# gongweibao/FleetX

Hardware: AMD Instinct MI355X
Metric: tokens/sec (whole node) GPT-3 6.7B hybrid-parallel at 1/2/4/8 MI355X (higher is better)
Workload: dtype bf16; 1 GPU; model=gpt3-6.7B, global_batch=8, seq_len=1024, parallelism=dp1, micro_batch=8, hip_graph=True, grad_reduce_dtype=float32, recompute=False

## Files before the change

csrc/kernels/norm_eltwise.hip:

```cpp
#include "fx_api.h"
#include "fx_common.h"

namespace {

struct DropCfg {
  uint32_t klo, khi, thr;
  float scale;
  int enabled;
  const uint64_t* salt;
};

__device__ __forceinline__ DropCfg resolve_drop(DropCfg d) {
  if (d.enabled && d.salt != nullptr) {
    const uint64_t k = salt_key(((uint64_t)d.khi << 32) | d.klo, *d.salt);
    d.klo = (uint32_t)k;
    d.khi = (uint32_t)(k >> 32);
  }
  return d;
}

__device__ __forceinline__ float drop_apply(float v, uint64_t idx, const DropCfg& d) {
  if (!d.enabled) return v;
  uint32_t h = elem_rand_pair(idx, d.klo, d.khi);
  uint32_t r = (idx & 1) ? (h >> 16) : (h & 0xffffu);
// ... 287 lines not shown
    const uint16_t* __restrict__ gamma, const uint16_t* __restrict__ ds_in,
    uint16_t* __restrict__ ds_out, uint16_t* __restrict__ dx_out, int rows, int h,
    int rows_per_group, float* __restrict__ part, DropCfg drop_) {
  constexpr int NG = 4 / WPR;
  __shared__ float red[4 * 512 * VPT];
  __shared__ float xs[2][4][2];
  const DropCfg drop = resolve_drop(drop_);
  const int lane = threadIdx.x & 63, w = threadIdx.x >> 6;
  const int grp = w / WPR, half = w % WPR;
  const int hw = h / WPR, cbase = half * hw;
  const int r0 = min(rows, (blockIdx.x * NG + grp) * rows_per_group);
  const int r1 = min(rows, r0 + rows_per_group);
  uint4 gp[VPT];
  float ag[VPT][8], ab[VPT][8], ax[DB ? VPT : 1][8];
#pragma unroll
  for (int i = 0; i < VPT; ++i) {
    const int c = (i * 64 + lane) * 8;
    gp[i] = (!MASK || c < hw) ? *reinterpret_cast<const uint4*>(gamma + cbase + c)
                              : make_uint4(0, 0, 0, 0);
#pragma unroll
    for (int j = 0; j < 8; ++j) {
      ag[i][j] = ab[i][j] = 0.f;
      if (DB) ax[i][j] = 0.f;
    }
  }
  for (int k = 0; k < rows_per_group; ++k) {
    const int r = r0 + k;
    const bool live = r < r1;
    if (WPR == 1 && !live) break;
    const size_t base = (size_t)(live ? r : 0) * h + cbase;
    uint4 ca[VPT], cd[VPT], cr[VPT];
    float mean = 0.f, rstd = 0.f, s1 = 0.f, s2 = 0.f;
    if (live) {
#pragma unroll
      for (int i = 0; i < VPT; ++i) {
        const int c = (i * 64 + lane) * 8;
        if (MASK && c >= hw) continue;
        ca[i] = *reinterpret_cast<const uint4*>(s + base + c);
        cd[i] = *reinterpret_cast<const uint4*>(dy + base + c);
      }
      if (ds_in) {
#pragma unroll
        for (int i = 0; i < VPT; ++i) {
          const int c = (i * 64 + lane) * 8;
          if (MASK && c >= hw) continue;
          cr[i] = *reinterpret_cast<const uint4*>(ds_in + base + c);
        }
      }
      mean = mean_in[r];
      rstd = rstd_in[r];
#pragma unroll
      for (int i = 0; i < VPT; ++i) {
        const int c = (i * 64 + lane) * 8;
        if (MASK && c >= hw) continue;
        float a[8], d[8], g[8];
        unpack8<T>(ca[i], a);
        unpack8<T>(cd[i], d);
        unpack8<T>(gp[i], g);
#pragma unroll
        for (int j = 0; j < 8; ++j) {
          const float xh = (a[j] - mean) * rstd, gd = d[j] * g[j];
          s1 += gd;
          s2 += gd * xh;
          ag[i][j] += d[j] * xh;
          ab[i][j] += d[j];
        }
      }
    }
    s1 = wave_sum(s1);
    s2 = wave_sum(s2);
    if constexpr (WPR > 1) {
      if (lane == 0) {
        xs[k & 1][w][0] = s1;
        xs[k & 1][w][1] = s2;
      }
      __syncthreads();
      s1 = xs[k & 1][WPR * grp][0];
      s2 = xs[k & 1][WPR * grp][1];
#pragma unroll
      for (int q = 1; q < WPR; ++q) {
        s1 += xs[k & 1][WPR * grp + q][0];
        s2 += xs[k & 1][WPR * grp + q][1];
      }
    }
    if (!live) continue;
    const float m1 = s1 / h, m2 = s2 / h;
#pragma unroll
    for (int i = 0; i < VPT; ++i) {
      const int c = (i * 64 + lane) * 8;
      if (MASK && c >= hw) continue;
      float a[8], d[8], g[8], o[8];
      unpack8<T>(ca[i], a);
      unpack8<T>(cd[i], d);
      unpack8<T>(gp[i], g);
#pragma unroll
      for (int j = 0; j < 8; ++j) o[j] = rstd * (d[j] * g[j] - m1 - (a[j] - mean) * rstd * m2);
      if (ds_in) {
        float rr[8];
        unpack8<T>(cr[i], rr);
#pragma unroll
        for (int j = 0; j < 8; ++j) o[j] += rr[j];
      }
      store8<T>(ds_out + base + c, o);
      if (drop.enabled) {
        drop_apply8(o, base + c, drop);
        store8<T>(dx_out + base + c, o);
      } else if (dx_out != ds_out) {
        store8<T>(dx_out + base + c, o);
      }
      if (DB) {
#pragma unroll
        for (int j = 0; j < 8; ++j) ax[i][j] += round_to<T>(o[j]);
      }
    }
  }
#pragma unroll
  for (int arr = 0; arr < (DB ? 3 : 2); ++arr) {
    __syncthreads();
#pragma unroll
    for (int i = 0; i < VPT; ++i) {
      const int c = (i * 64 + lane) * 8;
      if (MASK && c >= hw) continue;
#pragma unroll
      for (int j = 0; j < 8; ++j)
        red[grp * h + cbase + c + j] = arr == 0 ? ag[i][j] : arr == 1 ? ab[i][j] : ax[DB ? i : 0][j];
    }
    __syncthreads();
    float* out = part + ((size_t)arr * gridDim.x + blockIdx.x) * h;
    for (int c = threadIdx.x; c < h; c += 256) {
      float v = red[c];
#pragma unroll
      for (int q = 1; q < NG; ++q) v += red[q * h + c];
      out[c] = v;
    }
  }
}

struct LnColsOut {
  float* f32[3];
  uint16_t* t16[3];
  int acc[3];
};
template <typename T>
__global__ __launch_bounds__(256) void ln_cols_finalize_kernel(const float* __restrict__ part,
                                                               int G, int h, LnColsOut f) {
  __shared__ float tr[8][132];
  const int arr = blockIdx.y;
  const float* p = part + (size_t)arr * G * h;
  const int q = threadIdx.x & 31, sr = threadIdx.x >> 5;
  const int c0 = blockIdx.x * 128 + q * 4;
  floatx4 acc = {0.f, 0.f, 0.f, 0.f};
  if (c0 < h) {
    for (int k0 = sr; k0 < G; k0 += 128) {
      floatx4 v[16];
#pragma unroll
      for (int u = 0; u < 16; ++u) {
        const int k = k0 + 8 * u;
        v[u] = k < G ? *reinterpret_cast<const floatx4*>(p + (size_t)k * h + c0)
                     : floatx4{0.f, 0.f, 0.f, 0.f};
      }
#pragma unroll
      for (int u = 0; u < 16; ++u) acc += v[u];
    }
  }
#pragma unroll
  for (int j = 0; j < 4; ++j) tr[sr][q * 4 + j] = acc[j];
// ... 438 lines not shown
    }
#undef LNM_CASE
  } else {
    FX_DISPATCH_T(dtype, add_ln_fwd_generic<T><<<grid, block, 0, st>>>(
                             X, B, R, G, Be, S, Y, mean, rstd, rows, h, eps, d));
  }
#undef LN_CASE
}

extern "C" void fx_ln_bwd_row(int dtype, const void* dy, const void* s, const float* mean,
                              const float* rstd, const void* gamma, const void* ds_in,
                              void* ds_out, void* dx_out, int rows, int h, float p, uint64_t key,
                              const void* salt, hipStream_t st) {
  DropCfg d = make_drop(p, key, salt);
  dim3 grid((rows + 3) / 4), block(256);
  auto DY = (const uint16_t*)dy;
  auto S = (const uint16_t*)s;
  auto G = (const uint16_t*)gamma;
  auto DI = (const uint16_t*)ds_in;
  auto DS = (uint16_t*)ds_out;
  auto DX = (uint16_t*)dx_out;
#define LNB_CASE(V)                                                                       \
  case V:                                                                                 \
    FX_DISPATCH_T(dtype, ln_bwd_row_kernel<T, V><<<grid, block, 0, st>>>(                 \
                             DY, S, mean, rstd, G, DI, DS, DX, rows, h, d));              \
    break;
  if (h % 512 == 0 && h / 512 <= 8) {
    switch (h / 512) {
      LNB_CASE(1) LNB_CASE(2) LNB_CASE(3) LNB_CASE(4) LNB_CASE(5) LNB_CASE(6) LNB_CASE(7)
      LNB_CASE(8)
      default:
        FX_DISPATCH_T(dtype, ln_bwd_row_generic<T><<<grid, block, 0, st>>>(
                                 DY, S, mean, rstd, G, DI, DS, DX, rows, h, d));
    }
  } else if (h % 8 == 0 && h < 8 * 512) {
#define LNBM_CASE(V)                                                                      \
  case V:                                                                                 \
    FX_DISPATCH_T(dtype, ln_bwd_row_kernel<T, V, true><<<grid, block, 0, st>>>(           \
                             DY, S, mean, rstd, G, DI, DS, DX, rows, h, d));              \
    break;
    switch ((h + 511) / 512) {
      LNBM_CASE(1) LNBM_CASE(2) LNBM_CASE(3) LNBM_CASE(4) LNBM_CASE(5) LNBM_CASE(6)
      LNBM_CASE(7) LNBM_CASE(8)
    }
#undef LNBM_CASE
  } else {
    FX_DISPATCH_T(dtype, ln_bwd_row_generic<T><<<grid, block, 0, st>>>(
                             DY, S, mean, rstd, G, DI, DS, DX, rows, h, d));
  }
#undef LNB_CASE
}

static int ln_cols_wpr(int h) { return h <= 1536 ? 1 : h <= 3072 ? 2 : 4; }
static int ln_cols_rows_per_group(int rows, int h) {
  const int ng = 4 / ln_cols_wpr(h);
  int rpg = (rows + 512 * ng - 1) / (512 * ng);
  return rpg < 2 ? 2 : rpg;
}
extern "C" int fx_ln_bwd_cols_blocks(int rows, int h, int max_h) {
  if (rows <= 0 || h > (max_h < 4096 ? max_h : 4096) || h % (8 * ln_cols_wpr(h))) return 0;
  const int ng = 4 / ln_cols_wpr(h), rpg = ln_cols_rows_per_group(rows, h);
  return (rows + ng * rpg - 1) / (ng * rpg);
}

extern "C" int fx_ln_bwd_cols(int dtype, const void* dy, const void* s, const float* mean,
                              const float* rstd, const void* gamma, const void* ds_in,
                              void* ds_out, void* dx_out, int rows, int h, float p, uint64_t key,
                              float* part, int with_dbias, float* fg, void* tg, int accg,
                              float* fb, void* tb, int accb, float* fx, void* tx, int accx,
                              const void* salt, hipStream_t st) {
  const int G = fx_ln_bwd_cols_blocks(rows, h, 4096);
  if (G == 0) return -1;
  const int wpr = ln_cols_wpr(h), hw = h / wpr;
  const int rpg = ln_cols_rows_per_group(rows, h);
  DropCfg d = make_drop(p, key, salt);
  auto DY = (const uint16_t*)dy;
  auto S = (const uint16_t*)s;
  auto GM = (const uint16_t*)gamma;
  auto DI = (const uint16_t*)ds_in;
  auto DS = (uint16_t*)ds_out;
  auto DX = (uint16_t*)dx_out;
  const int vpt = (hw + 511) / 512;
  const bool mask = hw % 512 != 0;
#define LNC_GO(V, W, M, DB)                                                                   \
  FX_DISPATCH_T(dtype, ln_bwd_cols_kernel<T, V, W, M, DB><<<G, 256, 0, st>>>(                 \
                           DY, S, mean, rstd, GM, DI, DS, DX, rows, h, rpg, part, d))
#define LNC_M(V, W)                                                                           \
  if (mask) {                                                                                 \
    if (with_dbias) { LNC_GO(V, W, true, true); } else { LNC_GO(V, W, true, false); }         \
  } else {                                                                                    \
    if (with_dbias) { LNC_GO(V, W, false, true); } else { LNC_GO(V, W, false, false); }       \
  }
#define LNC_V(V)                                                                              \
  case V:                                                                                     \
    if (wpr == 1) { LNC_M(V, 1) } else if (wpr == 2) { LNC_M(V, 2) } else { LNC_M(V, 4) }     \
    break;
  switch (vpt) {
    LNC_V(1) LNC_V(2) LNC_V(3)
    default: return -1;
  }
#undef LNC_V
#undef LNC_M
#undef LNC_GO
  LnColsOut f;
  f.f32[0] = fg; f.f32[1] = fb; f.f32[2] = fx;
  f.t16[0] = (uint16_t*)tg; f.t16[1] = (uint16_t*)tb; f.t16[2] = (uint16_t*)tx;
  f.acc[0] = accg; f.acc[1] = accb; f.acc[2] = accx;
  dim3 grid((h + 127) / 128, with_dbias ? 3 : 2);
  FX_DISPATCH_T(dtype, ln_cols_finalize_kernel<T><<<grid, 256, 0, st>>>(part, G, h, f));
  return 0;
}

extern "C" void fx_coltile_partial(int dtype, int mode, const void* a, const void* b,
                                   const float* mean, const float* rstd, float* p0, float* p1,
                                   int rows, int cols, int splits, hipStream_t st, int* cnt,
                                   float* f0, void* t0, int acc0, float* f1, void* t1, int acc1) {
  const ColFin fin = make_fin(cnt, f0, t0, acc0, f1, t1, acc1);
  int rps = (rows + splits - 1) / splits;
  dim3 grid((cols + 127) / 128, splits), block(256);
  auto A = (const uint16_t*)a;
  auto B = (const uint16_t*)b;
  if (mode == 0) {
    FX_DISPATCH_T(dtype, coltile_partial_kernel<T, 0><<<grid, block, 0, st>>>(
                             A, B, mean, rstd, p0, p1, rows, cols, rps, fin));
  } else {
    FX_DISPATCH_T(dtype, coltile_partial_kernel<T, 1><<<grid, block, 0, st>>>(
                             A, B, mean, rstd, p0, p1, rows, cols, rps, fin));
  }
}

extern "C" void fx_coltile_finalize(int dtype, const float* part, int splits, int cols,
                                    float* out_f32, void* out_t, int accumulate, hipStream_t st) {
  dim3 grid((cols + 255) / 256), block(256);
  FX_DISPATCH_T(dtype, coltile_finalize_kernel<T><<<grid, block, 0, st>>>(
                           part, splits, cols, out_f32, (uint16_t*)out_t, accumulate));
}

extern "C" void fx_bias_gelu_fwd(int dtype, int erf, const void* x, const void* bias, void* y,
                                 long n, int cols, hipStream_t st) {
  long n8 = n / 8;
  if (erf) {
    FX_DISPATCH_T(dtype, bias_gelu_fwd_kernel<T, true><<<grid_for(n8), 256, 0, st>>>(
                             (const uint16_t*)x, (const uint16_t*)bias, (uint16_t*)y, n8, cols));
  } else {
    FX_DISPATCH_T(dtype, bias_gelu_fwd_kernel<T, false><<<grid_for(n8), 256, 0, st>>>(
                             (const uint16_t*)x, (const uint16_t*)bias, (uint16_t*)y, n8, cols));
  }
}

extern "C" void fx_bias_gelu_bwd(int dtype, int erf, const void* dy, const void* x,
                                 const void* bias, void* dx, float* part, int rows, int cols,
                                 int splits, hipStream_t st, int* cnt, float* out_f32,
                                 void* out_t, int acc) {
  const ColFin fin = make_fin(cnt, out_f32, out_t, acc, nullptr, nullptr, 0);
  int rps = (rows + splits - 1) / splits;
  dim3 grid((cols + 127) / 128, splits), block(256);
  if (erf) {
    FX_DISPATCH_T(dtype, bias_gelu_bwd_kernel<T, true><<<grid, block, 0, st>>>(
                             (const uint16_t*)dy, (const uint16_t*)x, (const uint16_t*)bias,
                             (uint16_t*)dx, part, rows, cols, rps, fin));
  } else {
    FX_DISPATCH_T(dtype, bias_gelu_bwd_kernel<T, false><<<grid, block, 0, st>>>(
                             (const uint16_t*)dy, (const uint16_t*)x, (const uint16_t*)bias,
                             (uint16_t*)dx, part, rows, cols, rps, fin));
  }
}

extern "C" void fx_bias_dropout_add_fwd(int dtype, const void* x, const void* bias,
                                        const void* residual, void* out, long n, int cols, float p,
                                        uint64_t key, const void* salt, hipStream_t st) {
  DropCfg d = make_drop(p, key, salt);
  long n8 = n / 8;
  FX_DISPATCH_T(dtype, bias_dropout_add_fwd_kernel<T><<<grid_for(n8), 256, 0, st>>>(
                           (const uint16_t*)x, (const uint16_t*)bias, (const uint16_t*)residual,
                           (uint16_t*)out, n8, cols, d));
}

extern "C" void fx_dropout_bwd_colsum(int dtype, const void* dout, void* dx, float* part,
                                      int rows, int cols, int splits, float p, uint64_t key,
                                      const void* salt, hipStream_t st, int* cnt,
                                      float* out_f32, void* out_t, int acc) {
  const ColFin fin = make_fin(cnt, out_f32, out_t, acc, nullptr, nullptr, 0);
  DropCfg d = make_drop(p, key, salt);
  int rps = (rows + splits - 1) / splits;
  dim3 grid((cols + 127) / 128, splits), block(256);
  FX_DISPATCH_T(dtype, dropout_bwd_colsum_kernel<T><<<grid, block, 0, st>>>(
// ... 11 lines not shown
```

fleetx_amd/models/language_model/gpt/model.py:

```python
import math

import torch
import torch.nn as nn

from .... import ops
from ....parallel import layers as L
from ....parallel import mappings as M
from ....parallel import topology as topo
from ....parallel.linear import fused_mlp
from ....parallel.recompute import recompute
from ....parallel.rng import get_rng_state_tracker


class GPTConfig:
    def __init__(self, vocab_size=50304, hidden_size=1024, num_layers=24, num_attention_heads=16,
                 ffn_hidden_size=None, hidden_dropout_prob=0.1, attention_probs_dropout_prob=0.1,
                 max_position_embeddings=1024, type_vocab_size=16, initializer_range=0.02,
                 use_recompute=False, recompute_granularity=None, sequence_parallel=False,
                 layer_norm_eps=1e-5, fused_linear=False, no_recompute_layers=None,
                 fused_lm_head_ce=False, dtype=torch.float32, **unused):
        self.vocab_size = vocab_size
        self.hidden_size = hidden_size
        self.num_layers = num_layers
        self.num_attention_heads = num_attention_heads
        self.ffn_hidden_size = ffn_hidden_size or 4 * hidden_size
        self.hidden_dropout_prob = hidden_dropout_prob
        self.attention_probs_dropout_prob = attention_probs_dropout_prob
        self.max_position_embeddings = max_position_embeddings
        self.type_vocab_size = type_vocab_size
        self.initializer_range = initializer_range
        self.use_recompute = use_recompute
        self.recompute_granularity = recompute_granularity or ("full" if use_recompute else None)
        self.sequence_parallel = sequence_parallel and topo.mp_world_size() > 1
        self.layer_norm_eps = layer_norm_eps
        self.no_recompute_layers = set(no_recompute_layers or [])
        self.dtype = dtype
        self.head_dim = hidden_size // num_attention_heads
        self.fused_lm_head_ce = bool(fused_lm_head_ce)

    @classmethod
    def from_model_config(cls, cfg, dtype=torch.float32):
        keys = ["vocab_size", "hidden_size", "num_layers", "num_attention_heads", "ffn_hidden_size",
                "hidden_dropout_prob", "attention_probs_dropout_prob", "max_position_embeddings",
                "type_vocab_size", "initializer_range", "use_recompute", "recompute_granularity",
                "sequence_parallel", "no_recompute_layers", "layer_norm_eps", "fused_lm_head_ce"]
        kw = {k: cfg[k] for k in keys if k in cfg and cfg[k] is not None}
        return cls(dtype=dtype, **kw)


def _key(stream):
    return get_rng_state_tracker().next_key(stream)


class GPTEmbeddings(nn.Module):
    def __init__(self, cfg):
        super().__init__()
        self.cfg = cfg
        self.word_embeddings = L.VocabParallelEmbedding(cfg.vocab_size, cfg.hidden_size,
                                                        std=cfg.initializer_range,
                                                        name="embeddings.word", dtype=cfg.dtype)
        self.position_embeddings = nn.Parameter(L.init_full_then_slice(
            (cfg.max_position_embeddings, cfg.hidden_size), cfg.initializer_range,
            "embeddings.position", dtype=cfg.dtype))
        self.position_embeddings.sequence_parallel = cfg.sequence_parallel

    def forward(self, input_ids, position_ids=None):
        b, s = input_ids.shape
        if position_ids is None:
            position_ids = torch.arange(s, device=input_ids.device).unsqueeze(0).expand(b, s)
        sp = self.cfg.sequence_parallel
        if sp:
            input_ids = input_ids.t()
            position_ids = position_ids.t()
        if topo.mp_world_size() == 1:
            x = ops.embedding(input_ids, self.word_embeddings.weight, position_ids,
                              self.position_embeddings, 0)
        else:
            x = self.word_embeddings(input_ids)
            if sp:
                x = M.reduce_scatter_seq(x)
                pos = ops.embedding(M._split(position_ids, topo.mp_group(), 0),
                                    self.position_embeddings)
            else:
                x = M.reduce_from_mp(x)
                pos = ops.embedding(position_ids, self.position_embeddings)
            x = x + pos
        p = self.cfg.hidden_dropout_prob if self.training else 0.0
        if p > 0:
            x = ops.dropout(x, p, _key("local_seed" if sp else "global_seed"))
        return x


class GPTAttention(nn.Module):
    def __init__(self, cfg, idx):
        super().__init__()
        self.cfg = cfg
        t = topo.mp_world_size()
        assert cfg.num_attention_heads % t == 0
        self.heads = cfg.num_attention_heads // t
        self.head_dim = cfg.head_dim
        std = cfg.initializer_range
        self.qkv_proj = L.ColumnParallelLinear(cfg.hidden_size, 3 * cfg.hidden_size, bias=True,
                                               sequence_parallel=cfg.sequence_parallel, std=std,
                                               name="layers.%d.attn.qkv" % idx, dtype=cfg.dtype)
        self.out_proj = L.RowParallelLinear(cfg.hidden_size, cfg.hidden_size, bias=True,
                                            skip_bias_add=True,
                                            sequence_parallel=cfg.sequence_parallel, std=std,
                                            name="layers.%d.attn.out" % idx, dtype=cfg.dtype)

    def core_attn(self, qkv, key):
        cfg = self.cfg
        p = cfg.attention_probs_dropout_prob if self.training else 0.0
        if cfg.sequence_parallel:
            s, b = qkv.shape[0], qkv.shape[1]
            qkv5 = qkv.view(s, b, self.heads, 3, self.head_dim).transpose(0, 1)
        else:
            b, s = qkv.shape[0], qkv.shape[1]
            qkv5 = qkv.view(b, s, self.heads, 3, self.head_dim)
        o = ops.flash_attention_qkvpacked(qkv5, causal=True, dropout_p=p, key=key)
        if cfg.sequence_parallel:
            return o.transpose(0, 1).reshape(s, b, self.heads * self.head_dim)
        return o.reshape(b, s, self.heads * self.head_dim)

    def forward(self, x):
        qkv = self.qkv_proj(x)
        key = _key("local_seed") if (self.training and self.cfg.attention_probs_dropout_prob > 0) else 0
        if self.cfg.recompute_granularity == "core_attn" and self.training:
            o = recompute(self.core_attn, qkv, key)
        else:
            o = self.core_attn(qkv, key)
        return self.out_proj(o)


class GPTMLP(nn.Module):
    def __init__(self, cfg, idx):
        super().__init__()
        std = cfg.initializer_range
        self.fc1 = L.ColumnParallelLinear(cfg.hidden_size, cfg.ffn_hidden_size, bias=True,
                                          skip_bias_add=True,
                                          sequence_parallel=cfg.sequence_parallel, std=std,
                                          name="layers.%d.mlp.fc1" % idx, dtype=cfg.dtype)
        self.fc2 = L.RowParallelLinear(cfg.ffn_hidden_size, cfg.hidden_size, bias=True,
                                       skip_bias_add=True, sequence_parallel=cfg.sequence_parallel,
                                       std=std, name="layers.%d.mlp.fc2" % idx, dtype=cfg.dtype)
        self.fc1.sp_chunk_major = self.fc2.sp_chunk_major = bool(cfg.sequence_parallel)

    def forward(self, x):
        if topo.mp_world_size() == 1 and type(self.fc1) is L.ColumnParallelLinear \
                and type(self.fc2) is L.RowParallelLinear:
            return fused_mlp(x, self.fc1.weight, self.fc1.bias, self.fc2.weight), self.fc2.bias
        y, b = self.fc1(x)
        y = ops.bias_gelu(y, b, approximate=True)
        return self.fc2(y)


class GPTDecoderLayer(nn.Module):

    def __init__(self, cfg, idx):
        super().__init__()
        self.cfg = cfg
        self.idx = idx
        self.ln1 = ops.FusedLayerNorm(cfg.hidden_size, cfg.layer_norm_eps, dtype=cfg.dtype)
        self.attn = GPTAttention(cfg, idx)
        self.ln2 = ops.FusedLayerNorm(cfg.hidden_size, cfg.layer_norm_eps, dtype=cfg.dtype)
        self.mlp = GPTMLP(cfg, idx)
        if cfg.sequence_parallel:
            L.mark_sequence_parallel(self.ln1)
            L.mark_sequence_parallel(self.ln2)

    def _attn_block(self, x):
        return self.attn(self.ln1(x))

    def _attn_block_out(self, x):
        return self._attn_block(x)[0]

    def _forward(self, x):
        cfg = self.cfg
        p = cfg.hidden_dropout_prob if self.training else 0.0
        stream = "local_seed" if cfg.sequence_parallel else "global_seed"
        if cfg.recompute_granularity == "full_attn" and self.training:
            a, ab = recompute(self._attn_block_out, x), self.attn.out_proj.bias
        else:
            x, h1 = ops.layer_norm_keep_input(x, self.ln1.weight, self.ln1.bias, self.ln1.eps)
            a, ab = self.attn(h1)
        k1 = _key(stream) if p > 0 else 0
        x2, h2 = ops.add_layer_norm(a, ab, x, self.ln2.weight, self.ln2.bias, self.ln2.eps, p, k1)
        m, mb = self.mlp(h2)
        k2 = _key(stream) if p > 0 else 0
        return ops.bias_dropout_add(m, mb, x2, p, k2)

    def forward(self, x):
        if (self.cfg.recompute_granularity == "full" and self.training
                and self.idx not in self.cfg.no_recompute_layers):
            return recompute(self._forward, x)
        return self._forward(x)


class GPTModel(nn.Module):

    def __init__(self, cfg, layer_range=None, has_embedding=True, has_final_ln=True):
        super().__init__()
        self.cfg = cfg
        start, end = layer_range if layer_range is not None else (0, cfg.num_layers)
        self.embeddings = GPTEmbeddings(cfg) if has_embedding else None
        self.layers = nn.ModuleList([GPTDecoderLayer(cfg, i) for i in range(start, end)])
        self.final_ln = ops.FusedLayerNorm(cfg.hidden_size, cfg.layer_norm_eps,
                                           dtype=cfg.dtype) if has_final_ln else None
        if has_final_ln and cfg.sequence_parallel:
            L.mark_sequence_parallel(self.final_ln)

    def forward(self, input_ids=None, position_ids=None, hidden=None):
        x = self.embeddings(input_ids, position_ids) if self.embeddings is not None else hidden
        for layer in self.layers:
            x = layer(x)
        if self.final_ln is not None:
            x = self.final_ln(x)
        return x


class GPTForPretraining(nn.Module):

    def __init__(self, cfg):
        super().__init__()
        self.cfg = cfg
        self.gpt = GPTModel(cfg)
        emb = self.gpt.embeddings
        if emb is not None:
            emb.word_embeddings.weight._fx_fused_wgrad_ok = True
            emb.word_embeddings.weight._fx_grad_parts = 2
            emb.position_embeddings._fx_fused_wgrad_ok = True

    def forward(self, input_ids, position_ids=None):
        h = self.gpt(input_ids, position_ids)
        w = self.gpt.embeddings.word_embeddings.weight
        if self.cfg.fused_lm_head_ce and self.training:
            return L.parallel_lm_head_input(h, w, sequence_parallel=self.cfg.sequence_parallel)
        logits = L.parallel_lm_logits(h, w, parallel_output=True,
                                      sequence_parallel=self.cfg.sequence_parallel)
        return logits


class GPTPretrainingCriterion(nn.Module):

    def __init__(self, cfg=None):
        super().__init__()
        self.seq_first = bool(cfg is not None and cfg.sequence_parallel)

    def forward(self, logits, labels, loss_mask):
        if self.seq_first:
            labels, loss_mask = labels.t(), loss_mask.t()
        g = topo.get_hcg().get_model_parallel_group()
        if isinstance(logits, L.HeadInput):
            from ....parallel.linear import linear
            from ....ops import lm_head_ce
            hi = logits
            vocab_start = topo.mp_rank() * hi.weight.shape[0]
            if lm_head_ce.supported(hi.h2, hi.weight):
                return lm_head_ce.lm_head_cross_entropy(
                    hi.h2, hi.weight, labels.reshape(-1), loss_mask.reshape(-1),
                    group=g if g.nranks > 1 else None, vocab_start=vocab_start)
            logits = linear(hi.h2, hi.weight)
        vocab_start = topo.mp_rank() * logits.shape[-1]
        ce = ops.softmax_cross_entropy(logits, labels, group=g if g.nranks > 1 else None,
                                       vocab_start=vocab_start)
        mask = loss_mask.reshape(-1).float()
        return (ce.reshape(-1) * mask).sum() / mask.sum()


def num_params(cfg):
    l, h, V, s = cfg.num_layers, cfg.hidden_size, cfg.vocab_size, cfg.max_position_embeddings
    return 12 * l * h * h * (1 + 13.0 / (12 * h) + (V + s) / (12.0 * l * h))


def flops_per_token(cfg, seq_len):
    l, h, V = cfg.num_layers, cfg.hidden_size, cfg.vocab_size
    return 72.0 * l * h * h * (1 + seq_len / (6.0 * h) + V / (12.0 * h * l))
```

fleetx_amd/ops/norm.py:

```python
import os

import torch

from . import _lib
from ..parallel import grad_sink as sink, rng as _rng


_TICKETS = {}


def colsum_tickets(device, cols):
    st = torch.cuda.current_stream(device).cuda_stream
    need = 32 * ((cols + 127) // 128)
    t = _TICKETS.get(st)
    if t is None or t.numel() < need:
        t = torch.zeros(max(4096, need), dtype=torch.int32, device=device)
        _TICKETS[st] = t
    return t.data_ptr()


_TARGET_KW = (("f0", "t0", "acc0"), ("f1", "t1", "acc1"))


def _coltile(mode, x, aux, rows, cols, targets):
    k = _lib.kernels()
    splits = k.coltile_splits(rows, cols)
    p0 = torch.empty(splits, cols, device=x.device, dtype=torch.float32)
    p1 = torch.empty_like(p0) if mode == 0 else None
    fin = {}
    for (kf, kt, ka), (f32, t16, acc) in zip(_TARGET_KW, targets):
        if f32:
            fin[kf], fin[ka] = f32, acc
        else:
            fin[kt] = t16
    k.coltile_partial(_lib.dt_code(x.dtype), mode, x.data_ptr(), *aux, p0.data_ptr(),
                      _lib.ptr(p1), rows, cols, splits, _lib.stream(),
                      cnt=colsum_tickets(x.device, cols), **fin)


def _col_target(prm, direct, cols, like):
    if direct:
        mg, acc = sink.open_write(prm)
        return (mg.data_ptr(), 0, int(acc)), None
    g = torch.empty(cols, device=like.device, dtype=like.dtype)
    return (0, g.data_ptr(), 0), g


def col_sum(x, cols):
    if not _lib.vec8_ok(cols, x):
        return x.reshape(-1, cols).float().sum(0).to(x.dtype)
    out = torch.empty(cols, device=x.device, dtype=x.dtype)
    _coltile(1, x, (0, 0, 0), x.numel() // cols, cols, [(0, out.data_ptr(), 0)])
    return out


def col_sum_f32(x, dst, accumulate=False):
    cols = dst.numel()
    x = x.contiguous()
    if not _lib.vec8_ok(cols, x):
        sink.store_or_add(dst, x.reshape(-1, cols).float().sum(0).view_as(dst), accumulate)
        return dst
    if dst.dtype != torch.float32 or not dst.is_contiguous():
        raise ValueError("col_sum_f32: dst must be contiguous fp32")
    _coltile(1, x, (0, 0, 0), x.numel() // cols, cols, [(dst.data_ptr(), 0, int(accumulate))])
    return dst


def _dropout_ref(x, p, key):
    if p <= 0.0:
        return x
    m = _rng.keep_mask(x.shape, p, key, x.device)
    return torch.where(m, x * (1.0 / (1.0 - p)), torch.zeros_like(x))


def _ln_bwd_cols_max_h():
    mode = os.environ.get("FLEETX_LN_BWD_FUSED", "1")
    return {"0": 0, "2": 4096}.get(mode, 1536)


def _ln_bwd_cols(k, dc, dy, s, mean, rstd, weight, ctx, ds_in, ds, dx, rows, h):
    G = k.ln_bwd_cols_blocks(rows, h, 4096)
    with_db = bool(ctx.has_bias)
    part = torch.empty(3 if with_db else 2, G, h, device=dy.device, dtype=torch.float32)
    prms = (weight, ctx.lnbias, ctx.bias if with_db else None)
    outs, grads = [], []
    for prm in prms:
        t, g = ((0, 0, 0), None) if prm is None else \
            _col_target(prm, sink.fused(prm, fp32_contiguous=True), h, dy)
        outs.append(t)
        grads.append(g)
    (fg, tg, ag), (fb, tb, ab), (fx, tx, ax) = outs
    rc = k.ln_bwd_cols(dc, dy.data_ptr(), s.data_ptr(), mean.data_ptr(), rstd.data_ptr(),
                       weight.data_ptr(), _lib.ptr(ds_in), ds.data_ptr(), dx.data_ptr(), rows, h,
                       float(ctx.p), ctx.key, part.data_ptr(), int(with_db), fg, tg, ag, fb, tb,
                       ab, fx, tx, ax, _rng.device_salt_ptr(), _lib.stream())
    if rc != 0:
        raise RuntimeError("ln_bwd_cols: shape rows=%d h=%d not covered" % (rows, h))
    for prm, (f32, _, _) in zip(prms, outs):
        if f32:
            sink.close_write(prm)
    return grads


class _AddLayerNorm(torch.autograd.Function):
    @staticmethod
    def forward(ctx, x, bias, residual, weight, lnbias, eps, p, key, store_sum):
        h = x.shape[-1]
        rows = x.numel() // h
        ctx.p, ctx.key, ctx.has_bias, ctx.has_res = p, key, bias is not None, residual is not None
        ctx.h = h
        x = x.contiguous()
        if _lib.vec8_ok(h, x, bias, residual, weight, lnbias):
            k = _lib.kernels()
            fused = bias is not None or residual is not None or p > 0
            s = torch.empty_like(x) if fused else None
            y = torch.empty_like(x)
            mean = torch.empty(rows, device=x.device, dtype=torch.float32)
            rstd = torch.empty_like(mean)
            k.add_ln_fwd(_lib.dt_code(x.dtype), x.data_ptr(), _lib.ptr(bias), _lib.ptr(residual),
                         weight.data_ptr(), lnbias.data_ptr(), _lib.ptr(s), y.data_ptr(),
                         mean.data_ptr(), rstd.data_ptr(), rows, h, float(eps), float(p), key,
                         _rng.device_salt_ptr(), _lib.stream())
            s_saved = s if s is not None else x
            if s is None and store_sum:
                s = x
        else:
            v = x
            if bias is not None or residual is not None or p > 0:
                v = x.float() if bias is None else x.float() + bias.float()
                v = _dropout_ref(v, p, key)
                if residual is not None:
                    v = v + residual.float()
                v = v.to(x.dtype)
            s_saved = v
            s = v if (store_sum or bias is not None or residual is not None or p > 0) else None
            vf = v.float()
            mean = vf.mean(-1).reshape(-1)
            var = ((vf - mean.view(*vf.shape[:-1], 1)) ** 2).mean(-1).reshape(-1)
            rstd = torch.rsqrt(var + eps)
            y = ((vf - mean.view(*vf.shape[:-1], 1)) * rstd.view(*vf.shape[:-1], 1) * weight.float()
                 + lnbias.float()).to(x.dtype)
        ctx.save_for_backward(s_saved, mean, rstd, weight)
        ctx.lnbias, ctx.bias = lnbias, bias
        ctx.return_sum = s is not None
        if s is None:
            return y
        return s, y

    @staticmethod
    def backward(ctx, *grads):
        if ctx.return_sum:
            ds_in, dy = grads
        else:
            ds_in, dy = None, grads[0]
        s, mean, rstd, weight = ctx.saved_tensors
        h = ctx.h
        rows = s.numel() // h
        dy = dy.contiguous()
        if ds_in is not None:
            ds_in = ds_in.contiguous()
        if _lib.vec8_ok(h, dy, ds_in, s, weight):
            k = _lib.kernels()
            dc = _lib.dt_code(dy.dtype)
            ds = torch.empty_like(dy)
            dx = torch.empty_like(dy) if ctx.p > 0 else ds
            if k.ln_bwd_cols_blocks(rows, h, _ln_bwd_cols_max_h()) > 0:
                dw, db, dbias = _ln_bwd_cols(k, dc, dy, s, mean, rstd, weight, ctx, ds_in, ds, dx,
                                             rows, h)
                dres = ds if ctx.has_res else None
                return dx, dbias, dres, dw, db, None, None, None, None
            k.ln_bwd_row(dc, dy.data_ptr(), s.data_ptr(), mean.data_ptr(), rstd.data_ptr(),
                         weight.data_ptr(), _lib.ptr(ds_in), ds.data_ptr(), dx.data_ptr(), rows, h,
                         float(ctx.p), ctx.key, _rng.device_salt_ptr(), _lib.stream())
            direct = sink.fused(weight) and sink.fused(ctx.lnbias)
            (tw, dw), (tb, db) = (_col_target(prm, direct, h, dy) for prm in (weight, ctx.lnbias))
            _coltile(0, dy, (s.data_ptr(), mean.data_ptr(), rstd.data_ptr()), rows, h, [tw, tb])
            if direct:
                sink.close_write(weight)
                sink.close_write(ctx.lnbias)
            dbias = None
            if ctx.has_bias:
                if sink.fused(ctx.bias):
                    mg, acc = sink.open_write(ctx.bias)
                    col_sum_f32(dx, mg, acc)
                    sink.close_write(ctx.bias)
                else:
                    dbias = col_sum(dx, h)
        else:
            sf = s.float().reshape(rows, h)
            xh = (sf - mean.view(rows, 1)) * rstd.view(rows, 1)
            g = dy.float().reshape(rows, h) * weight.float()
            m1 = g.mean(-1, keepdim=True)
            m2 = (g * xh).mean(-1, keepdim=True)
            dsf = rstd.view(rows, 1) * (g - m1 - xh * m2)
            if ds_in is not None:
                dsf = dsf + ds_in.float().reshape(rows, h)
            ds = dsf.to(dy.dtype).reshape(dy.shape)
            dx = _dropout_ref(ds, ctx.p, ctx.key)
            dw = sink.deliver(weight, (dy.float().reshape(rows, h) * xh).sum(0), weight.dtype,
                              on_gpu=True)
            db = sink.deliver(ctx.lnbias, dy.float().reshape(rows, h).sum(0), weight.dtype,
                              on_gpu=True)
            dbias = None
            if ctx.has_bias:
                dbias = sink.deliver(ctx.bias, dx.float().reshape(rows, h).sum(0), dy.dtype,
                                     on_gpu=True)
        dres = ds if ctx.has_res else None
        return dx, dbias, dres, dw, db, None, None, None, None


def add_layer_norm(x, bias, residual, weight, lnbias, eps=1e-5, p=0.0, key=0):
    return _AddLayerNorm.apply(x, bias, residual, weight, lnbias, eps, p, key, True)


def layer_norm(x, weight, bias, eps=1e-5):
    return _AddLayerNorm.apply(x, None, None, weight, bias, eps, 0.0, 0, False)


def layer_norm_keep_input(x, weight, bias, eps=1e-5):
    return _AddLayerNorm.apply(x, None, None, weight, bias, eps, 0.0, 0, True)


class FusedLayerNorm(torch.nn.Module):

    def __init__(self, hidden, eps=1e-5, dtype=None, device=None):
        super().__init__()
        self.weight = torch.nn.Parameter(torch.ones(hidden, dtype=dtype, device=device))
        self.bias = torch.nn.Parameter(torch.zeros(hidden, dtype=dtype, device=device))
        self.weight._fx_fused_wgrad_ok = True
        self.bias._fx_fused_wgrad_ok = True
        self.eps = eps
        self.normalized_shape = (hidden,)

    def forward(self, x):
        return layer_norm(x, self.weight, self.bias, self.eps)
```

fleetx_amd/parallel/sharding.py:

```python
import contextlib

import torch
import torch.distributed as dist

from . import grad_sink as sink
from .grad_buffer import ALIGN, Category, _is_gloo, _round_up, default_decay_fn


def _free(t):
    if t.untyped_storage().size() != 0:
        t.untyped_storage().resize_(0)


def _alloc(t, numel):
    nbytes = numel * t.element_size()
    if t.untyped_storage().size() != nbytes:
        t.untyped_storage().resize_(nbytes)


def _in_backward():
    try:
        return torch._C._current_graph_task_id() != -1
    except AttributeError:
        return False
# ... 126 lines not shown
        for u in self.all_units:
            u.full_param = torch.zeros(u.numel, dtype=self.dtype, device=self.device)
            u.full_grad = torch.zeros(u.numel, dtype=torch.float32, device=self.device)
            for seg in u.segments:
                for n, p, o in seg.params:
                    view = u.full_param[o:o + p.numel()].view_as(p)
                    view.copy_(p.data)
                    p.data = view
                    p.main_grad = u.full_grad[o:o + p.numel()].view_as(p)
                    p.grad = None
                    p._fx_fresh = True
                    p._fx_fused_wgrad = bool(getattr(p, "_fx_fused_wgrad_ok", False)) and fused_wgrad
                    p._fx_unit = u
                    self.params.append((n, p))
            u.gathered = True
            u.grad_live = True
            self._writeback_shard(u)
            if self.shard_params:
                self._release_params(u)
            self._release_grads(u)
        self._install_hooks(model)

    def _piece(self, seg):
        return (seg.fend - seg.fstart) // self.nsh

    def _writeback_shard(self, u):
        for seg in u.segments:
            piece = self._piece(seg)
            lo = seg.fstart + self.rank * piece
            self.param_flat[seg.sstart:seg.send].copy_(u.full_param[lo:lo + piece])

    def _gather(self, u, async_op=True):
        if u.gathered:
            return
        _alloc(u.full_param, u.numel)
        works = []
        for seg in u.segments:
            out = u.full_param[seg.fstart:seg.fend]
            mine = self.param_flat[seg.sstart:seg.send]
            if self.gloo:
                parts = [torch.empty_like(mine) for _ in range(self.nsh)]
                dist.all_gather(parts, mine, group=self.shard_group.group)
                out.copy_(torch.cat(parts))
            else:
                w = dist.all_gather_into_tensor(out, mine, group=self.shard_group.group,
                                                async_op=async_op)
                if w is not None:
                    works.append(w)
        u.gather_works = works
        u.gathered = True

    def _wait_gather(self, u):
        for w in u.gather_works:
            w.wait()
        u.gather_works = []

    def _release_params(self, u):
        if not u.gathered:
            return
        self._wait_gather(u)
        if not self.shard_params:
            return
        _free(u.full_param)
        u.gathered = False

    def _alloc_grads(self, u):
        if u.grad_live:
            return
        _alloc(u.full_grad, u.numel)
        u.grad_live = True
        for seg in u.segments:
            for n, p, o in seg.params:
                p._fx_fresh = True
        u.ready = 0
        u.done = False

    def _release_grads(self, u):
        if u.grad_live:
            _free(u.full_grad)
            u.grad_live = False

    def _install_hooks(self, model):
        for u in self.units:
            self._hooks.append(u.module.register_forward_pre_hook(self._make_pre_fwd(u)))
            self._hooks.append(u.module.register_forward_hook(self._make_post_fwd(u)))
        if self.root is not None:
            self._hooks.append(model.register_forward_pre_hook(self._root_pre_fwd))
        for n, p in self.params:
            self._hooks.append(p.register_post_accumulate_grad_hook(self._accum_hook))
            p._fx_grad_ready = self._make_ready(p)

    def _root_pre_fwd(self, module, args):
        self._gather(self.root, async_op=False)
        self._wait_gather(self.root)
        if torch.is_grad_enabled():
            self._alloc_grads(self.root)
        if self.units and self.prefetch:
            self._gather(self.units[0])

    def _make_pre_fwd(self, u):
        def hook(module, args):
            self._gather(u)
            self._wait_gather(u)
            if self.prefetch and u.idx + 1 < len(self.units) and not _in_backward():
                self._gather(self.units[u.idx + 1])
        return hook

    def _make_post_fwd(self, u):
        def hook(module, args, output):
            if _in_backward():
                return output
            if torch.is_grad_enabled():
                outs = output if isinstance(output, (tuple, list)) else (output,)
                fired = [False]

                def pre_bwd(grad, u=u, fired=fired):
                    if not fired[0]:
                        fired[0] = True
                        self._pre_backward(u)
                    return grad
                for t in outs:
                    if torch.is_tensor(t) and t.requires_grad:
                        t.register_hook(pre_bwd)
            self._release_params(u)
            return output
        return hook

    def _pre_backward(self, u):
        self._gather(u)
        self._wait_gather(u)
        self._alloc_grads(u)
        if self.prefetch and u.idx >= 1:
            self._gather(self.units[u.idx - 1])

    def _accum_hook(self, param):
        sink.absorb(param)

    def _make_ready(self, p):
        def ready():
            u = p._fx_unit
            if u is self.root:
                return
            u.ready += 1
            if u.ready == len(u.named):
                self._unit_backward_done(u)
        return ready

    def _zero_missing(self, u):
        for seg in u.segments:
            prev = seg.fstart
            for n, p, o in seg.params:
                if p._fx_fresh:
                    p.main_grad.zero_()
                    p._fx_fresh = False
                if o > prev:
                    u.full_grad[prev:o].zero_()
                prev = o + p.numel()
            if seg.fend > prev:
                u.full_grad[prev:seg.fend].zero_()

    def _launch_rs(self, u):
        from .linear import join_wgrad_stream
        join_wgrad_stream()
        self._zero_missing(u)
        works, pieces = [], []
        for seg in u.segments:
# ... 48 lines not shown

    def zero_grad(self):
        for u in self.all_units:
            u.shard_fresh = True

    def finish(self):
        from .linear import join_wgrad_stream
        join_wgrad_stream()
        for u in self.units:
            if u.grad_live and not u.done:
                self._launch_rs(u)
                self._pending_rs.append(u)
        if self.root is not None and self.root.grad_live:
            self._launch_rs(self.root)
            self._pending_rs.append(self.root)
        self._drain()
        for u in self.all_units:
            if u.shard_fresh:
                for seg in u.segments:
                    self.grad_flat[seg.sstart:seg.send].zero_()
                u.shard_fresh = False
            self._release_params(u)
        data_world = self.nsh
        if self.dp_group is not None:
            dist.all_reduce(self.grad_flat, group=self.dp_group.group)
            data_world *= self.dp_group.nranks
        self.grad_flat.mul_(1.0 / data_world)
        if self.mp_group is not None:
            for c in self.category_list:
                if c.seq_parallel and c.end > c.start:
                    dist.all_reduce(self.grad_flat[c.start:c.end], group=self.mp_group.group)

    def owned_ranges(self):
        return [(c.start, c.end, c) for c in self.category_list]

    def allgather_params(self):
        if self.shard_params:
            return
        for u in self.all_units:
            self._wait_gather(u)
            works = []
            for seg in u.segments:
                out = u.full_param[seg.fstart:seg.fend]
                mine = self.param_flat[seg.sstart:seg.send]
                if self.gloo:
                    parts = [torch.empty_like(mine) for _ in range(self.nsh)]
                    dist.all_gather(parts, mine, group=self.shard_group.group)
                    out.copy_(torch.cat(parts))
                else:
                    works.append(dist.all_gather_into_tensor(out, mine,
                                                             group=self.shard_group.group,
                                                             async_op=True))
            u.gather_works = works

    def sync_params(self):
        for u in self.all_units:
            self._wait_gather(u)

    @contextlib.contextmanager
    def gathered(self, writeback=False):
        for u in self.all_units:
            self._gather(u, async_op=False)
            self._wait_gather(u)
        try:
            yield
        finally:
            for u in self.all_units:
                if writeback:
                    self._writeback_shard(u)
                self._release_params(u)

    def memory_report(self):
        full = sum(u.numel for u in self.all_units)
        esz = self.param_flat.element_size()
        return {"stage": self.shard_stage,
                "resident_param_bytes": (self.param_flat.numel() if self.shard_params
                                         else full) * esz,
                "shard_param_bytes": self.param_flat.numel() * esz,
                "shard_grad_bytes": self.grad_flat.numel() * 4,
                "unsharded_param_bytes": full * esz,
                "unsharded_grad_bytes": full * 4}

    def remove_hooks(self):
        for h in self._hooks:
            h.remove()
        self._hooks = []
```

Baseline: 28770 tokens/s.

## Fuse layer seams into add-layernorm and add wide multi-row LN backward kernel

Each transformer layer can now defer its final bias-dropout-add, so the next layer's ln1 (or the final LN) performs it inside a fused add_layer_norm. This removes one elementwise pass and one activation round trip per layer boundary. A new wide column-reduction LN backward kernel handles several rows per iteration when each row spans multiple waves, and the fused backward is enabled by default up to h=4096. This covers h=4096 here and adds register pressure plus more complex dispatch. set_materialize_grads(False) is added, with zero-filling when dy is None.

```diff
diff --git a/csrc/kernels/norm_eltwise.hip b/csrc/kernels/norm_eltwise.hip
--- a/csrc/kernels/norm_eltwise.hip
+++ b/csrc/kernels/norm_eltwise.hip
@@ -393,6 +393,276 @@
         s1 += xs[k & 1][WPR * grp + q][0];
         s2 += xs[k & 1][WPR * grp + q][1];
       }
+    }
+    if (!live) continue;
+    const float m1 = s1 / h, m2 = s2 / h;
+#pragma unroll
+    for (int i = 0; i < VPT; ++i) {
+      const int c = (i * 64 + lane) * 8;
+      if (MASK && c >= hw) continue;
+      float a[8], d[8], g[8], o[8];
+      unpack8<T>(ca[i], a);
+      unpack8<T>(cd[i], d);
+      unpack8<T>(gp[i], g);
+#pragma unroll
+      for (int j = 0; j < 8; ++j) o[j] = rstd * (d[j] * g[j] - m1 - (a[j] - mean) * rstd * m2);
+      if (ds_in) {
+        float rr[8];
+        unpack8<T>(cr[i], rr);
+#pragma unroll
+        for (int j = 0; j < 8; ++j) o[j] += rr[j];
+      }
+      store8<T>(ds_out + base + c, o);
+      if (drop.enabled) {
+        drop_apply8(o, base + c, drop);
+        store8<T>(dx_out + base + c, o);
+      } else if (dx_out != ds_out) {
+        store8<T>(dx_out + base + c, o);
+      }
+      if (DB) {
+#pragma unroll
+        for (int j = 0; j < 8; ++j) ax[i][j] += round_to<T>(o[j]);
+      }
+    }
+  }
+#pragma unroll
+  for (int arr = 0; arr < (DB ? 3 : 2); ++arr) {
+    __syncthreads();
+#pragma unroll
+    for (int i = 0; i < VPT; ++i) {
+      const int c = (i * 64 + lane) * 8;
+      if (MASK && c >= hw) continue;
+#pragma unroll
+      for (int j = 0; j < 8; ++j)
+        red[grp * h + cbase + c + j] = arr == 0 ? ag[i][j] : arr == 1 ? ab[i][j] : ax[DB ? i : 0][j];
+    }
+    __syncthreads();
+    float* out = part + ((size_t)arr * gridDim.x + blockIdx.x) * h;
+    for (int c = threadIdx.x; c < h; c += 256) {
+      float v = red[c];
+#pragma unroll
+      for (int q = 1; q < NG; ++q) v += red[q * h + c];
+      out[c] = v;
+    }
+  }
+}
+
+__device__ __forceinline__ void keep_packed(uint4& v) {
+  asm volatile("" : "+v"(v.x), "+v"(v.y), "+v"(v.z), "+v"(v.w));
+}
+
+template <typename T, int VPT, int WPR, bool MASK, bool DB, int RB>
+__global__ __launch_bounds__(256, 2) void ln_bwd_cols_wide_kernel(
+    const uint16_t* __restrict__ dy, const uint16_t* __restrict__ s,
+    const float* __restrict__ mean_in, const float* __restrict__ rstd_in,
+    const uint16_t* __restrict__ gamma, const uint16_t* __restrict__ ds_in,
+    uint16_t* __restrict__ ds_out, uint16_t* __restrict__ dx_out, int rows, int h,
+    int rows_per_group, float* __restrict__ part, DropCfg drop_) {
+  static_assert(WPR == 2 || WPR == 4, "one wave per row is ln_bwd_cols_kernel");
+  constexpr int NG = 4 / WPR;
+  __shared__ float red[4 * 512 * VPT];
+  __shared__ float xs[2][4][RB][2];
+  const DropCfg drop = resolve_drop(drop_);
+  const int lane = threadIdx.x & 63, w = __builtin_amdgcn_readfirstlane(threadIdx.x >> 6);
+  const int grp = w / WPR, half = w % WPR;
+  const int hw = h / WPR, cbase = half * hw;
+  const int r0 = min(rows, (blockIdx.x * NG + grp) * rows_per_group);
+  const int r1 = min(rows, r0 + rows_per_group);
+  uint4 gp[VPT];
+  float ag[VPT][8], ab[VPT][8], ax[DB ? VPT : 1][8];
+#pragma unroll
+  for (int i = 0; i < VPT; ++i) {
+    const int c = (i * 64 + lane) * 8;
+    gp[i] = (!MASK || c < hw) ? *reinterpret_cast<const uint4*>(gamma + cbase + c)
+                              : make_uint4(0, 0, 0, 0);
+#pragma unroll
+    for (int j = 0; j < 8; ++j) {
+      ag[i][j] = ab[i][j] = 0.f;
+      if (DB) ax[i][j] = 0.f;
+    }
+  }
+  const int rlast = min(rows, (blockIdx.x * NG + NG - 1) * rows_per_group);
+  const int nlast = min(rows, rlast + rows_per_group) - rlast;
+  const int nfull = nlast / RB * RB;
+  int par = 0;
+  for (int k = 0; k < nfull; k += RB, par ^= 1) {
+    const int rb0 = __builtin_amdgcn_readfirstlane(r0 + k);
+    const int rend = __builtin_amdgcn_readfirstlane(r1);
+    uint4 ca[RB][VPT], cd[RB][VPT], cr[RB][VPT];
+    float mean[RB], rstd[RB], s1[RB], s2[RB];
+#pragma unroll
+    for (int b = 0; b < RB; ++b) {
+      const size_t base = (size_t)(rb0 + b) * h + cbase;
+      const uint16_t* sp = s + base;
+      const uint16_t* dp = dy + base;
+#pragma unroll
+      for (int i = 0; i < VPT; ++i) {
+        const unsigned c = (i * 64 + lane) * 8;
+        if (MASK && c >= hw) continue;
+        ca[b][i] = *reinterpret_cast<const uint4*>(sp + c);
+        cd[b][i] = *reinterpret_cast<const uint4*>(dp + c);
+      }
+    }
+    if (ds_in) {
+#pragma unroll
+      for (int b = 0; b < RB; ++b) {
+        const uint16_t* rp = ds_in + (size_t)(rb0 + b) * h + cbase;
+#pragma unroll
+        for (int i = 0; i < VPT; ++i) {
+          const unsigned c = (i * 64 + lane) * 8;
+          if (MASK && c >= hw) continue;
+          cr[b][i] = *reinterpret_cast<const uint4*>(rp + c);
+        }
+      }
+    }
+#pragma unroll
+    for (int b = 0; b < RB; ++b) {
+      mean[b] = rstd[b] = s1[b] = s2[b] = 0.f;
+      if (rb0 + b >= rend) continue;
+      mean[b] = mean_in[rb0 + b];
+      rstd[b] = rstd_in[rb0 + b];
+#pragma unroll
+      for (int i = 0; i < VPT; ++i) {
+        const int c = (i * 64 + lane) * 8;
+        if (MASK && c >= hw) continue;
+        float a[8], d[8], g[8];
+        unpack8<T>(ca[b][i], a);
+        unpack8<T>(cd[b][i], d);
+        unpack8<T>(gp[i], g);
+#pragma unroll
+        for (int j = 0; j < 8; ++j) {
+          const float xh = (a[j] - mean[b]) * rstd[b], gd = d[j] * g[j];
+          s1[b] += gd;
+          s2[b] += gd * xh;
+          ag[i][j] += d[j] * xh;
+          ab[i][j] += d[j];
+        }
+      }
+    }
+#pragma unroll
+    for (int b = 0; b < RB; ++b) {
+      s1[b] = wave_sum(s1[b]);
+      s2[b] = wave_sum(s2[b]);
+    }
+    if (lane == 0) {
+#pragma unroll
+      for (int b = 0; b < RB; ++b) {
+        xs[par][w][b][0] = s1[b];
+        xs[par][w][b][1] = s2[b];
+      }
+    }
+    __syncthreads();
+#pragma unroll
+    for (int b = 0; b < RB; ++b) {
+      s1[b] = xs[par][WPR * grp][b][0];
+      s2[b] = xs[par][WPR * grp][b][1];
+#pragma unroll
+      for (int q = 1; q < WPR; ++q) {
+        s1[b] += xs[par][WPR * grp + q][b][0];
+        s2[b] += xs[par][WPR * grp + q][b][1];
+      }
+    }
+#pragma unroll
+    for (int b = 0; b < RB; ++b) {
+#pragma unroll
+      for (int i = 0; i < VPT; ++i) {
+        keep_packed(ca[b][i]);
+        keep_packed(cd[b][i]);
+      }
+    }
+#pragma unroll
+    for (int b = 0; b < RB; ++b) {
+      if (rb0 + b >= rend) continue;
+      const size_t base = (size_t)(rb0 + b) * h + cbase;
+      uint16_t* dsp = ds_out + base;
+      uint16_t* dxp = dx_out + base;
+      const float m1 = s1[b] / h, m2 = s2[b] / h;
+#pragma unroll
+      for (int i = 0; i < VPT; ++i) {
+        const unsigned c = (i * 64 + lane) * 8;
+        if (MASK && c >= hw) continue;
+        float a[8], d[8], g[8], o[8];
+        unpack8<T>(ca[b][i], a);
+        unpack8<T>(cd[b][i], d);
+        unpack8<T>(gp[i], g);
+#pragma unroll
+        for (int j = 0; j < 8; ++j)
+          o[j] = rstd[b] * (d[j] * g[j] - m1 - (a[j] - mean[b]) * rstd[b] * m2);
+        if (ds_in) {
+          float rr[8];
+          unpack8<T>(cr[b][i], rr);
+#pragma unroll
+          for (int j = 0; j < 8; ++j) o[j] += rr[j];
+        }
+        store8<T>(dsp + c, o);
+        if (drop.enabled) {
+          drop_apply8(o, base + c, drop);
+          store8<T>(dxp + c, o);
+        } else if (dx_out != ds_out) {
+          store8<T>(dxp + c, o);
+        }
+        if (DB) {
+#pragma unroll
+          for (int j = 0; j < 8; ++j) ax[i][j] += round_to<T>(o[j]);
+        }
+      }
+    }
+  }
+  for (int k = nfull; k < rows_per_group; ++k, par ^= 1) {
+    const int r = r0 + k;
+    const bool live = r < r1;
+    const size_t base = (size_t)(live ? r : 0) * h + cbase;
+    uint4 ca[VPT], cd[VPT], cr[VPT];
+    float mean = 0.f, rstd = 0.f, s1 = 0.f, s2 = 0.f;
+    if (live) {
+#pragma unroll
+      for (int i = 0; i < VPT; ++i) {
+        const int c = (i * 64 + lane) * 8;
+        if (MASK && c >= hw) continue;
+        ca[i] = *reinterpret_cast<const uint4*>(s + base + c);
+        cd[i] = *reinterpret_cast<const uint4*>(dy + base + c);
+      }
+      if (ds_in) {
+#pragma unroll
+        for (int i = 0; i < VPT; ++i) {
+          const int c = (i * 64 + lane) * 8;
+          if (MASK && c >= hw) continue;
+          cr[i] = *reinterpret_cast<const uint4*>(ds_in + base + c);
+        }
+      }
+      mean = mean_in[r];
+      rstd = rstd_in[r];
+#pragma unroll
+      for (int i = 0; i < VPT; ++i) {
+        const int c = (i * 64 + lane) * 8;
+        if (MASK && c >= hw) continue;
+        float a[8], d[8], g[8];
+        unpack8<T>(ca[i], a);
+        unpack8<T>(cd[i], d);
+        unpack8<T>(gp[i], g);
+#pragma unroll
+        for (int j = 0; j < 8; ++j) {
+          const float xh = (a[j] - mean) * rstd, gd = d[j] * g[j];
+          s1 += gd;
+          s2 += gd * xh;
+          ag[i][j] += d[j] * xh;
+          ab[i][j] += d[j];
+        }
+      }
+    }
+    s1 = wave_sum(s1);
+    s2 = wave_sum(s2);
+    if (lane == 0) {
+      xs[par][w][0][0] = s1;
+      xs[par][w][0][1] = s2;
+    }
+    __syncthreads();
+    s1 = xs[par][WPR * grp][0][0];
+    s2 = xs[par][WPR * grp][0][1];
+#pragma unroll
+    for (int q = 1; q < WPR; ++q) {
+      s1 += xs[par][WPR * grp + q][0][0];
+      s2 += xs[par][WPR * grp + q][0][1];
     }
     if (!live) continue;
     const float m1 = s1 / h, m2 = s2 / h;
@@ -997,26 +1267,39 @@
   auto DX = (uint16_t*)dx_out;
   const int vpt = (hw + 511) / 512;
   const bool mask = hw % 512 != 0;
-#define LNC_GO(V, W, M, DB)                                                                   \
-  FX_DISPATCH_T(dtype, ln_bwd_cols_kernel<T, V, W, M, DB><<<G, 256, 0, st>>>(                 \
-                           DY, S, mean, rstd, GM, DI, DS, DX, rows, h, rpg, part, d))
-#define LNC_M(V, W)                                                                           \
+#define LNC_ARGS DY, S, mean, rstd, GM, DI, DS, DX, rows, h, rpg, part, d
+#define LNC_ONE(V, M, DB) \
+  FX_DISPATCH_T(dtype, ln_bwd_cols_kernel<T, V, 1, M, DB><<<G, 256, 0, st>>>(LNC_ARGS))
+#define LNC_WIDE(V, W, M, DB)                                                                 \
+  FX_DISPATCH_T(dtype, ln_bwd_cols_wide_kernel<T, V, W, M, DB, ((V) == 3 || (M)) ? 2 : 4>     \
+                           <<<G, 256, 0, st>>>(LNC_ARGS))
+#define LNC_MD(GO, ...)                                                                       \
   if (mask) {                                                                                 \
-    if (with_dbias) { LNC_GO(V, W, true, true); } else { LNC_GO(V, W, true, false); }         \
+    if (with_dbias) { GO(__VA_ARGS__, true, true); } else { GO(__VA_ARGS__, true, false); }   \
   } else {                                                                                    \
-    if (with_dbias) { LNC_GO(V, W, false, true); } else { LNC_GO(V, W, false, false); }       \
-  }
-#define LNC_V(V)                                                                              \
-  case V:                                                                                     \
-    if (wpr == 1) { LNC_M(V, 1) } else if (wpr == 2) { LNC_M(V, 2) } else { LNC_M(V, 4) }     \
-    break;
-  switch (vpt) {
-    LNC_V(1) LNC_V(2) LNC_V(3)
-    default: return -1;
-  }
-#undef LNC_V
-#undef LNC_M
-#undef LNC_GO
+    if (with_dbias) { GO(__VA_ARGS__, false, true); } else { GO(__VA_ARGS__, false, false); } \
+  }
+  if (wpr == 1) {
+    switch (vpt) {
+      case 1: LNC_MD(LNC_ONE, 1) break;
+      case 2: LNC_MD(LNC_ONE, 2) break;
+      case 3: LNC_MD(LNC_ONE, 3) break;
+      default: return -1;
+    }
+  } else if (wpr == 2) {
+    switch (vpt) {
+      case 2: LNC_MD(LNC_WIDE, 2, 2) break;
+      case 3: LNC_MD(LNC_WIDE, 3, 2) break;
+      default: return -1;
+    }
+  } else {
+    if (vpt != 2) return -1;
+    LNC_MD(LNC_WIDE, 2, 4)
+  }
+#undef LNC_MD
+#undef LNC_WIDE
+#undef LNC_ONE
+#undef LNC_ARGS
   LnColsOut f;
   f.f32[0] = fg; f.f32[1] = fb; f.f32[2] = fx;
   f.t16[0] = (uint16_t*)tg; f.t16[1] = (uint16_t*)tb; f.t16[2] = (uint16_t*)tx;
diff --git a/fleetx_amd/models/language_model/gpt/model.py b/fleetx_amd/models/language_model/gpt/model.py
--- a/fleetx_amd/models/language_model/gpt/model.py
+++ b/fleetx_amd/models/language_model/gpt/model.py
@@ -1,4 +1,5 @@
 import math
+import os
 
 import torch
 import torch.nn as nn
@@ -52,6 +53,10 @@
     return get_rng_state_tracker().next_key(stream)
 
 
+def _layer_seam():
+    return os.environ.get("FLEETX_LAYER_SEAM", "1") != "0"
+
+
 class GPTEmbeddings(nn.Module):
     def __init__(self, cfg):
         super().__init__()
@@ -174,11 +179,24 @@
     def _attn_block_out(self, x):
         return self._attn_block(x)[0]
 
-    def _forward(self, x):
+    def _recomputed(self):
+        return (self.cfg.recompute_granularity == "full" and self.training
+                and self.idx not in self.cfg.no_recompute_layers)
+
+    def joins_seam(self):
+        return not self._recomputed() and not (
+            self.cfg.recompute_granularity == "full_attn" and self.training) and not getattr(
+            self, "_fx_params_released", False)
+
+    def _forward(self, x, pending=None, defer=False):
         cfg = self.cfg
         p = cfg.hidden_dropout_prob if self.training else 0.0
         stream = "local_seed" if cfg.sequence_parallel else "global_seed"
-        if cfg.recompute_granularity == "full_attn" and self.training:
+        if pending is not None:
+            x, h1 = ops.add_layer_norm(*pending[:3], self.ln1.weight, self.ln1.bias,
+                                       self.ln1.eps, *pending[3:])
+            a, ab = self.attn(h1)
+        elif cfg.recompute_granularity == "full_attn" and self.training:
             a, ab = recompute(self._attn_block_out, x), self.attn.out_proj.bias
         else:
             x, h1 = ops.layer_norm_keep_input(x, self.ln1.weight, self.ln1.bias, self.ln1.eps)
@@ -187,13 +205,14 @@
         x2, h2 = ops.add_layer_norm(a, ab, x, self.ln2.weight, self.ln2.bias, self.ln2.eps, p, k1)
         m, mb = self.mlp(h2)
         k2 = _key(stream) if p > 0 else 0
+        if defer:
+            return m, mb, x2, p, k2
         return ops.bias_dropout_add(m, mb, x2, p, k2)
 
-    def forward(self, x):
-        if (self.cfg.recompute_granularity == "full" and self.training
-                and self.idx not in self.cfg.no_recompute_layers):
+    def forward(self, x, pending=None, defer=False):
+        if self._recomputed():
             return recompute(self._forward, x)
-        return self._forward(x)
+        return self._forward(x, pending, defer)
 
 
 class GPTModel(nn.Module):
@@ -211,9 +230,18 @@
 
     def forward(self, input_ids=None, position_ids=None, hidden=None):
         x = self.embeddings(input_ids, position_ids) if self.embeddings is not None else hidden
-        for layer in self.layers:
-            x = layer(x)
-        if self.final_ln is not None:
+        seam = _layer_seam() and not self.cfg.sequence_parallel
+        pending = None
+        for i, layer in enumerate(self.layers):
+            nxt = self.layers[i + 1] if i + 1 < len(self.layers) else None
+            defer = seam and layer.joins_seam() and (
+                nxt.joins_seam() if nxt is not None else self.final_ln is not None)
+            out = layer(x, pending, defer)
+            x, pending = (None, out) if defer else (out, None)
+        if pending is not None:
+            ln = self.final_ln
+            _, x = ops.add_layer_norm(*pending[:3], ln.weight, ln.bias, ln.eps, *pending[3:])
+        elif self.final_ln is not None:
             x = self.final_ln(x)
         return x
 
diff --git a/fleetx_amd/ops/norm.py b/fleetx_amd/ops/norm.py
--- a/fleetx_amd/ops/norm.py
+++ b/fleetx_amd/ops/norm.py
@@ -73,9 +73,15 @@
     return torch.where(m, x * (1.0 / (1.0 - p)), torch.zeros_like(x))
 
 
-def _ln_bwd_cols_max_h():
+_WIDE_DEFAULT = {2: True, 4: True}
+
+
+def _ln_bwd_cols_max_h(h):
     mode = os.environ.get("FLEETX_LN_BWD_FUSED", "1")
-    return {"0": 0, "2": 4096}.get(mode, 1536)
+    if mode in ("0", "2"):
+        return {"0": 0, "2": 4096}[mode]
+    wpr = 1 if h <= 1536 else 2 if h <= 3072 else 4
+    return 4096 if _WIDE_DEFAULT.get(wpr, True) else 1536
 
 
 def _ln_bwd_cols(k, dc, dy, s, mean, rstd, weight, ctx, ds_in, ds, dx, rows, h):
@@ -109,6 +115,7 @@
         rows = x.numel() // h
         ctx.p, ctx.key, ctx.has_bias, ctx.has_res = p, key, bias is not None, residual is not None
         ctx.h = h
+        ctx.set_materialize_grads(False)
         x = x.contiguous()
         if _lib.vec8_ok(h, x, bias, residual, weight, lnbias):
             k = _lib.kernels()
@@ -156,6 +163,8 @@
         s, mean, rstd, weight = ctx.saved_tensors
         h = ctx.h
         rows = s.numel() // h
+        if dy is None:
+            dy = torch.zeros_like(s)
         dy = dy.contiguous()
         if ds_in is not None:
             ds_in = ds_in.contiguous()
@@ -164,7 +173,7 @@
             dc = _lib.dt_code(dy.dtype)
             ds = torch.empty_like(dy)
             dx = torch.empty_like(dy) if ctx.p > 0 else ds
-            if k.ln_bwd_cols_blocks(rows, h, _ln_bwd_cols_max_h()) > 0:
+            if k.ln_bwd_cols_blocks(rows, h, _ln_bwd_cols_max_h(h)) > 0:
                 dw, db, dbias = _ln_bwd_cols(k, dc, dy, s, mean, rstd, weight, ctx, ds_in, ds, dx,
                                              rows, h)
                 dres = ds if ctx.has_res else None
diff --git a/fleetx_amd/parallel/sharding.py b/fleetx_amd/parallel/sharding.py
--- a/fleetx_amd/parallel/sharding.py
+++ b/fleetx_amd/parallel/sharding.py
@@ -232,6 +232,7 @@
 
     def _install_hooks(self, model):
         for u in self.units:
+            u.module._fx_params_released = True
             self._hooks.append(u.module.register_forward_pre_hook(self._make_pre_fwd(u)))
             self._hooks.append(u.module.register_forward_hook(self._make_post_fwd(u)))
         if self.root is not None:
@@ -446,6 +447,8 @@
                 "unsharded_grad_bytes": full * 4}
 
     def remove_hooks(self):
+        for u in self.units:
+            u.module._fx_params_released = False
         for h in self._hooks:
             h.remove()
         self._hooks = []
```

Result: no change. 28910 tokens/s (median of 6 runs) (+0.5%).
